# ehgus8/alpha-zero

Measured on AMD Instinct MI355X. Metric: selfplay_games_per_sec, higher is better.
Workload: dtype bf16

## Files before the change

alpha-zero_amd/azk/__init__.py:

```python
import ctypes as C
import math
import os
import subprocess

import numpy as np

_HERE = os.path.dirname(os.path.abspath(__file__))
_CSRC = os.path.join(os.path.dirname(_HERE), "csrc")
LIB_PATH = os.path.join(_HERE, "libazk.so")

ABI_VERSION = 4

SYMBOLS = [
    "azk_abi_version", "azk_last_error", "azk_create", "azk_destroy", "azk_geometry", "azk_reset_games",
    "azk_set_positions", "azk_begin_search", "azk_step_select", "azk_step_expand_backup", "azk_step",
    "azk_root_stats", "azk_root_children", "azk_export_tree", "azk_advance", "azk_get_positions",
    "azk_get_counters", "azk_reset_counters", "azk_check_device_error", "azk_gen_noise",
    "azk_rules_legal_moves", "azk_rules_legal_mask", "azk_rules_apply_move", "azk_rules_undo_move",
    "azk_rules_check_winner", "azk_rules_canonical", "azk_softmax_rows",
    "azk_step_tree", "azk_step_gather", "azk_recycle_finished", "azk_nn_patch_embed", "azk_nn_cls_attention", "azk_nn_patch_embed_scores", "azk_nn_cls_pool", "azk_debug_stamps", "azk_debug_stamps_raw", "azk_emit_finished", "azk_clear_cache", "azk_nn_heads_finalize", "azk_nn_layernorm_rows",
    "azk_vanilla_set_rng", "azk_vanilla_get_rng", "azk_vanilla_search", "azk_nn_embed_pool",
    "azk_nn_gemm_rows", "azk_nn_layernorm_sum", "azk_nn_heads_finalize_sum", "azk_nn_ln_heads",
    "azk_leaf_source_of", "azk_nn_embed_pool_leaves", "azk_nn_embed_pool_compact", "azk_nn_embed_pool_compact_leaves",
    "azk_nn_embed_fold", "azk_nn_embed_fold_leaves", "azk_nnx_embed_fold", "azk_nnx_embed_fold_leaves",
# ... 54 lines not shown
    if not torch.cuda.is_available():
        raise AzkError("no GPU visible: the azk engine runs only on an MI355X (no CPU fallback)")
    return torch


def _stream():
    import torch
    return C.c_void_p(torch.cuda.current_stream().cuda_stream)


def _p(t):
    return C.c_void_p(t.data_ptr()) if t is not None else None


def _np(a):
    return a.ctypes.data_as(C.c_void_p) if a is not None else None


def _ok(rc, name):
    if rc != 0:
        raise AzkError(f"{name} failed ({rc})")


class Engine:

    def __init__(self, game, n_games, max_sims, size=None, device=0, leaf_dtype="float32", arena_nodes=0, cache_entries=0,
                 cache_shared=False, leaves_per_step=1, tree_reuse=0):
        torch = _torch()
        self.torch = torch
        self.L = lib()
        self.game = game
        cfg = Config()
        cfg.game = GAME_ID[game]
        cfg.rows = cfg.cols = int(size or 0)
        cfg.n_games, cfg.max_sims, cfg.device, cfg.arena_nodes = int(n_games), int(max_sims), int(device), int(arena_nodes)
        cfg.cache_entries = int(cache_entries)
        cfg.cache_shared = 1 if (cache_shared and cache_entries) else 0
        self.cache_shared = bool(cfg.cache_shared)
        self.K = max(1, int(leaves_per_step))
        cfg.leaves_per_step = self.K
        self.tree_reuse = int(tree_reuse)
        cfg.tree_reuse = self.tree_reuse
        cfg.leaf_dtype = LEAF_BF16 if leaf_dtype in ("bfloat16", "bf16", torch.bfloat16) else LEAF_F32
        self.device = torch.device("cuda", device)
        torch.cuda.set_device(self.device)
        h = C.c_void_p()
        rc = self.L.azk_create(C.byref(cfg), C.byref(h))
        if rc != 0:
            raise AzkError(f"azk_create failed ({rc}): {self.L.azk_last_error(None).decode()}")
        self.h = h
        vals = [C.c_int32() for _ in range(5)]
        self._chk(self.L.azk_geometry(self.h, *[C.byref(v) for v in vals]))
        self.planes, self.rows, self.cols, self.action_dim, self.state_dim = [v.value for v in vals]
        self.G, self.max_sims = int(n_games), int(max_sims)
        tdt = torch.bfloat16 if cfg.leaf_dtype == LEAF_BF16 else torch.float32
        dev = self.device
        self.slots = self.G * self.K
        self.leaf_boards = torch.zeros((self.slots, self.planes, self.rows, self.cols), dtype=tdt, device=dev)
        self.n_leaf = torch.zeros(1, dtype=torch.int32, device=dev)
        self.pi = torch.zeros((self.G, self.action_dim), dtype=torch.float64, device=dev)
        self.q = torch.zeros(self.G, dtype=torch.float64, device=dev)
        self.root_visit = torch.zeros(self.G, dtype=torch.int32, device=dev)
        self.chosen = torch.zeros(self.G, dtype=torch.int32, device=dev)
        self.winner = torch.zeros(self.G, dtype=torch.int32, device=dev)
        self.done = torch.zeros(self.G, dtype=torch.int32, device=dev)
        self._noise = None
        self.cache_entries = int(cache_entries)
# ... 795 lines not shown
```

alpha-zero_amd/csrc/azk_device.h:

```cpp
#pragma once
#include <hip/hip_runtime.h>
#include <stdint.h>

#define AZK_WAVE 64
#define AZK_KIND_TTT 0
#define AZK_KIND_C4 1
#define AZK_KIND_GOMOKU 2

struct GameDesc {
    int kind, rows, cols, rc, planes, win_len, action_dim, state_dim;
    unsigned inv_cols;
};

__device__ __forceinline__ int azk_action_idx(const GameDesc &g, int cell) {
    return g.kind == AZK_KIND_C4 ? cell % g.cols : cell;
}

__device__ __forceinline__ int azk_lane() { return threadIdx.x & 63; }

__device__ __forceinline__ int uniform_i32(int v) { return __builtin_amdgcn_readfirstlane(v); }

__device__ __forceinline__ void azk_wave_sync() {
    __builtin_amdgcn_fence(__ATOMIC_RELEASE, "wavefront");
    __builtin_amdgcn_wave_barrier();
// ... 148 lines not shown

__device__ __forceinline__ unsigned long long py_tuple2_hash(int r, int c) {
    const unsigned long long P1 = 11400714785074694791ULL, P2 = 14029467366897019727ULL, P5 = 2870177450012600261ULL;
    unsigned long long acc = P5;
    acc += (unsigned long long)r * P2; acc = (acc << 31) | (acc >> 33); acc *= P1;
    acc += (unsigned long long)c * P2; acc = (acc << 31) | (acc >> 33); acc *= P1;
    acc += 2ULL ^ (P5 ^ 3527539ULL);
    if (acc == ~0ULL) return 1546275796ULL;
    return acc;
}

struct MoveScratch {
    uint32_t *bits;
    uint16_t *pref;
    int16_t *ord;
    uint16_t *tabA, *tabB;
    uint32_t *claim;
    int table_size;
};

struct AzkNoHook { __device__ __forceinline__ void operator()() const {} };

__device__ __forceinline__ int azk_valid_moves_small(const uint8_t *b, const GameDesc &g, int16_t *moves) {
    const int lane = azk_lane();
    int n = 0;
    if (g.kind == AZK_KIND_TTT) {
        for (int base = 0; base < g.rc; base += AZK_WAVE) {
            int i = base + lane;
            bool emp = i < g.rc && b[i] == 0;
            unsigned long long m = __ballot(emp);
            if (emp) moves[n + __popcll(m & ((1ull << lane) - 1ull))] = (int16_t)i;
            n += __popcll(m);
        }
        __syncthreads();
        return n;
    }
    int cell = -1;
    if (lane < g.cols && b[lane] == 0) {
        for (int row = g.rows - 1; row >= 0; row--)
            if (b[row * g.cols + lane] == 0) { cell = row * g.cols + lane; break; }
    }
    unsigned long long m = __ballot(cell >= 0);
    if (cell >= 0) moves[__popcll(m & ((1ull << lane) - 1ull))] = (int16_t)cell;
    __syncthreads();
    return __popcll(m);
}

template <int KMAX = 7, typename Mid = AzkNoHook>
__device__ int azk_valid_moves_gomoku(const uint8_t *b, const GameDesc &g, int16_t *moves, const MoveScratch &ms, bool skip_set = false,
                                      long long *dbgv = nullptr, Mid &&mid = Mid()) {
    const int lane = azk_lane();
    int n = 0;
    const int R = g.rows, C = g.cols, rc = g.rc;
    const int nwords = (rc * 8 + 31) >> 5;
    long long s0 = dbgv ? clock64() : 0, s1 = 0, s2 = 0, s3 = 0;
    const unsigned inv = g.inv_cols;
    uint8_t code[KMAX];
#pragma unroll
    for (int k = 0; k < KMAX; k++) {
        const int e = lane + AZK_WAVE * k;
        code[k] = b[e < rc ? e : 0];
    }
    for (int w = lane; w < nwords; w += AZK_WAVE) ms.bits[w] = 0u;
    unsigned long long S[KMAX + 1], CL[KMAX], CR[KMAX];
    bool empty[KMAX];
#pragma unroll
    for (int k = 0; k < KMAX; k++) {
        S[k] = 0ull; CL[k] = 0ull; CR[k] = 0ull; empty[k] = false;
        if (AZK_WAVE * k >= rc) continue;
        const int e = lane + AZK_WAVE * k;
        const bool in = e < rc;
        const int r = (int)(((unsigned)(in ? e : 0) * inv) >> 16), c = (in ? e : 0) - r * C;
        S[k] = __ballot(in && (code[k] & 3));
        CL[k] = __ballot(c >= 1);
        CR[k] = __ballot(c <= C - 2);
        empty[k] = in && code[k] == 0;
    }
// ... 315 lines not shown
```

alpha-zero_amd/csrc/azk_engine.hip:

```cpp
#include <hip/hip_runtime.h>
#include <hip/hip_bf16.h>
#include <stdint.h>
#include <stdio.h>
#include <stdlib.h>
#include <string.h>
#include <string>
#include <vector>

#include "azk.h"
#include "azk_device.h"

namespace {

enum { CNT_SIMS = 0, CNT_SCANNED, CNT_TRACE, CNT_CREATED, CNT_LEAVES, CNT_TERMINAL, CNT_MOVES, CNT_CACHE_HITS, CNT_REUSED, CNT_CARRIED, CNT_N };

struct __attribute__((aligned(16))) NodeH { int N; float P; uint32_t meta; int fc; };
typedef float f32x4_a4 __attribute__((ext_vector_type(4), aligned(4)));

struct Dev {
    GameDesc g;
    int G, cap, path_cap, rc_pad, leaf_dtype, table_size, lds_bytes;
    int lds_off[12];
    int K;
    uint8_t *cells;
// ... 19 lines not shown
    int cache_shared;
    unsigned long long cache_mask;
    unsigned *cache_claim;
    unsigned *cache_stamp;
    unsigned long long *leaf_key;
    float *hit_logits, *hit_value;
    int16_t *traj_action;
    double *traj_pi;
    long long *emit_base;
    int *sims_done;
    int *budget;
    long long *counters;
    int *err;
    int ablate;
    long long *dbg;
};

struct ReuseDev {
    int mode;
    int words;
    int *chosen_node;
    unsigned long long *bits;
    unsigned *pre;
};

struct LdsView {
    uint8_t *board;
    int *path;
    int16_t *moves;
    float *e;
    int *cnt;
    double *cdf;
    MoveScratch ms;
};

__host__ __device__ inline int up16(int x) { return (x + 15) & ~15; }

__host__ __device__ inline int lds_layout(const GameDesc &g, int path_cap, int table_size, int *off) {
    int o = 0;
    off[0] = o; o += up16(g.rc);
    off[1] = o; o += up16(path_cap * 4);
    off[2] = o; o += up16(g.rc * 2);
    int ea = g.action_dim > g.rc ? g.action_dim : g.rc;
    off[3] = o; o += up16(ea * 4);
    off[4] = o; o += up16(ea * 4);
    off[5] = o; o += up16(ea * 8);
    int nwords = (g.rc * 8 + 31) >> 5;
    off[6] = o; o += up16((nwords > (table_size >> 5) + 2 ? nwords : (table_size >> 5) + 2) * 4);
    off[7] = o; o += up16(nwords * 2);
    off[8] = o; o += up16(g.rc * 2);
    off[9] = o; o += up16(table_size * 2);
    off[10] = o; o += up16(table_size * 2);
    off[11] = o; o += up16(table_size * 4);
    return o;
}

extern __shared__ __attribute__((aligned(16))) unsigned char azk_smem[];

__device__ __forceinline__ LdsView carve_at(const int *off, int table_size) {
    LdsView L;
    L.board = azk_smem + off[0];
    L.path = (int *)(azk_smem + off[1]);
    L.moves = (int16_t *)(azk_smem + off[2]);
    L.e = (float *)(azk_smem + off[3]);
    L.cnt = (int *)(azk_smem + off[4]);
    L.cdf = (double *)(azk_smem + off[5]);
    L.ms.bits = (uint32_t *)(azk_smem + off[6]);
    L.ms.pref = (uint16_t *)(azk_smem + off[7]);
    L.ms.ord = (int16_t *)(azk_smem + off[8]);
    L.ms.tabA = (uint16_t *)(azk_smem + off[9]);
    L.ms.tabB = (uint16_t *)(azk_smem + off[10]);
    L.ms.claim = (uint32_t *)(azk_smem + off[11]);
    L.ms.table_size = table_size;
    return L;
}

__device__ __forceinline__ LdsView carve(const GameDesc &g, int path_cap, int table_size) {
    int off[12];
    lds_layout(g, path_cap, table_size, off);
    LdsView L;
    L.board = azk_smem + off[0];
    L.path = (int *)(azk_smem + off[1]);
    L.moves = (int16_t *)(azk_smem + off[2]);
    L.e = (float *)(azk_smem + off[3]);
    L.cnt = (int *)(azk_smem + off[4]);
    L.cdf = (double *)(azk_smem + off[5]);
    L.ms.bits = (uint32_t *)(azk_smem + off[6]);
    L.ms.pref = (uint16_t *)(azk_smem + off[7]);
    L.ms.ord = (int16_t *)(azk_smem + off[8]);
    L.ms.tabA = (uint16_t *)(azk_smem + off[9]);
    L.ms.tabB = (uint16_t *)(azk_smem + off[10]);
    L.ms.claim = (uint32_t *)(azk_smem + off[11]);
    L.ms.table_size = table_size;
    return L;
}

__device__ __forceinline__ uint32_t meta_pack(int cell, int nch) { return ((uint32_t)(cell & 0xffff) << 16) | (uint32_t)nch; }
__device__ __forceinline__ int meta_cell(uint32_t m) { return (int)(m >> 16); }
__device__ __forceinline__ int meta_nch(uint32_t m) { return (int)(m & 0xffffu); }

__device__ __forceinline__ void count_add(const Dev &d, int which, int g, long long v) {
    atomicAdd((unsigned long long *)&d.counters[(size_t)which * d.G + g], (unsigned long long)v);
}

__device__ __forceinline__ void backup_path(const Dev &d, size_t base, const int *path, int depth, double value, bool undo_virtual_loss = false) {
    for (int i = azk_lane(); i <= depth; i += AZK_WAVE) {
        int nd = path[i];
        double sv = ((depth - i) & 1) ? -value : value;
        if (undo_virtual_loss) { d.W[base + nd] = (d.W[base + nd] + sv) + 1.0; continue; }
        d.H[base + nd].N += 1;
        d.W[base + nd] += sv;
    }
}

template <bool EXPAND, bool SELECT, bool DBG, bool MULTI = false, int KSL = 7>
__global__ __launch_bounds__(AZK_WAVE) void k_tree(Dev dd, const float *__restrict__ logits, const float *__restrict__ values) {
    const Dev &d = dd;
    const int ablate = DBG ? dd.ablate : 0;
    const int g = blockIdx.x;
    const int lane0 = azk_lane();
    const GameDesc &gd = d.g;
    const int A = gd.action_dim, rc = gd.rc;
    const size_t base = (size_t)g * (size_t)d.cap;
    LdsView L = carve_at(d.lds_off, d.table_size);
    const bool wrec = DBG && (ablate & 8192) != 0;
    const bool stamp = (ablate & 16) != 0 || wrec;
    long long t0 = stamp ? clock64() : 0, t1 = 0, t2 = 0, t3 = 0, t4 = 0;
    int rec_type = -1, rec_depth = 0, rec_nv = 0, rec_env = 0;
    int done_sims = MULTI ? d.sims_done[g] : 0;
    const int sim_target = MULTI ? d.budget[0] : 0, max_iter = MULTI ? d.budget[1] : 1;
    const int young = MULTI ? d.budget[2] : 0;
    const long long t_launch = MULTI && young > 0 ? (long long)wall_clock64() : 0;
    auto still_young = [&]() { return young <= 0 || (long long)wall_clock64() - t_launch < (long long)young; };
    for (int it = 0; it < max_iter; it++) {
    int lane = lane0;
    if (MULTI) asm volatile("" : "+v"(lane));
    if (MULTI && it > 0) __syncthreads();
    const bool vl = MULTI && d.K > 1;
    const int vi = g * d.K + (vl ? it : 0);

    const bool shared = d.cache_entries && d.cache_shared;
    int e_node, e_slot, e_depth, e_nv, e_top, e_centry, s_done, s_player, s_mc, s_rootf64, r_fc, r_N;
    uint32_t r_meta;
    unsigned cstamp;
    constexpr bool ONE_LOAD = EXPAND && SELECT && !MULTI;
    int uw = 0;
    if (ONE_LOAD) {
        const int *up = d.leaf_node + vi;
        up = lane == 1 ? d.leaf_slot + vi : up;
        up = lane == 2 ? d.leaf_depth + vi : up;
        up = lane == 3 ? d.leaf_nmoves + vi : up;
        up = lane == 4 ? d.arena_top + g : up;
        up = (lane == 5 && d.cache_entries) ? d.leaf_cache + vi : up;
        up = (lane == 6 && shared) ? (const int *)d.cache_stamp : up;
        up = lane == 7 ? d.done + g : up;
        up = lane == 8 ? d.to_move + g : up;
        up = lane == 9 ? d.move_count + g : up;
        up = lane == 10 ? d.root_f64 + g : up;
        up = lane == 11 ? &d.H[base].fc : up;
        up = lane == 12 ? &d.H[base].N : up;
        up = lane == 13 ? (const int *)&d.H[base].meta : up;
        uw = *up;
    } else {
        e_node = EXPAND ? d.leaf_node[vi] : -1; e_slot = EXPAND ? d.leaf_slot[vi] : 0; e_depth = EXPAND ? d.leaf_depth[vi] : 0;
        e_nv = EXPAND ? d.leaf_nmoves[vi] : 0; e_top = EXPAND ? d.arena_top[g] : 0;
        e_centry = (EXPAND && d.cache_entries) ? d.leaf_cache[vi] : -1;
        cstamp = shared ? d.cache_stamp[0] : 0u;
        s_done = SELECT ? d.done[g] : 1; s_player = SELECT ? d.to_move[g] : 0; s_mc = SELECT ? d.move_count[g] : 0;
        s_rootf64 = SELECT ? d.root_f64[g] : 0;
        r_fc = SELECT ? d.H[base].fc : -1; r_N = SELECT ? d.H[base].N : 0;
        r_meta = SELECT ? d.H[base].meta : 0u;
    }
    unsigned long long e_key = 0ull;
    if (EXPAND && shared) e_key = d.leaf_key[(size_t)vi * d.key_words + min(lane, d.key_words - 1)];
    const int e_path = EXPAND ? d.path[(size_t)vi * d.path_cap + min(lane, d.path_cap - 1)] : 0;
    int e_mv[KSL] = {};
    if (EXPAND) {
#pragma unroll
        for (int k4 = 0; k4 < KSL; k4++) e_mv[k4] = d.leaf_moves[(size_t)vi * rc + min(lane + AZK_WAVE * k4, rc - 1)];
    }
    constexpr int NCW = (KSL * AZK_WAVE / 4 + AZK_WAVE - 1) / AZK_WAVE;
    const int ncw = d.rc_pad >> 2;
    uint32_t s_cw[NCW] = {};
    if (SELECT) {
        const uint32_t *cw = (const uint32_t *)(d.cells + (size_t)g * d.rc_pad);
#pragma unroll
        for (int q = 0; q < NCW; q++) s_cw[q] = cw[min(lane + AZK_WAVE * q, ncw - 1)];
    }
    if (ONE_LOAD) {
        e_node = __builtin_amdgcn_readlane(uw, 0); e_slot = __builtin_amdgcn_readlane(uw, 1); e_depth = __builtin_amdgcn_readlane(uw, 2);
        e_nv = __builtin_amdgcn_readlane(uw, 3); e_top = __builtin_amdgcn_readlane(uw, 4);
        e_centry = d.cache_entries ? __builtin_amdgcn_readlane(uw, 5) : -1;
        cstamp = shared ? (unsigned)__builtin_amdgcn_readlane(uw, 6) : 0u;
        s_done = __builtin_amdgcn_readlane(uw, 7); s_player = __builtin_amdgcn_readlane(uw, 8); s_mc = __builtin_amdgcn_readlane(uw, 9);
        s_rootf64 = __builtin_amdgcn_readlane(uw, 10); r_fc = __builtin_amdgcn_readlane(uw, 11); r_N = __builtin_amdgcn_readlane(uw, 12);
        r_meta = (uint32_t)__builtin_amdgcn_readlane(uw, 13);
    }

    if (EXPAND) {
        const int node = uniform_i32(e_node);
        if (MULTI && node >= 0 && !(d.cache_entries && uniform_i32(e_centry) >= 0) && ((!vl && it > 0) || logits == nullptr)) {
            if (lane == 0) atomicExch(d.err, AZK_ERR_STATE);
            break;
        }
        if (node >= 0) {
            const bool xst = (ablate & 1024) != 0;
            long long x0 = 0, x1 = 0, x2 = 0, x3 = 0, x4 = 0;
            if (xst) { asm volatile("s_waitcnt vmcnt(0)" ::: "memory"); x0 = clock64(); }
            const int slot = uniform_i32(e_slot);
            const int depth = uniform_i32(e_depth);
            const int nv = uniform_i32(e_nv);
            if (wrec) rec_env = nv;
            const int centry = d.cache_entries ? uniform_i32(e_centry) : -1;
            const bool hit = d.cache_entries && centry >= 0;
            const size_t crow = shared ? (size_t)(hit ? centry : -(centry + 1)) : ((size_t)g * d.cache_entries + (hit ? centry : -(centry + 1)));
            const float *lg = hit ? (shared ? d.hit_logits + (size_t)vi * A : d.cache_logits + crow * A) : logits + (size_t)slot * A;
            unsigned claim_now = 0u;
            if (shared && !hit) claim_now = __hip_atomic_load(d.cache_claim + crow, __ATOMIC_RELAXED, __HIP_MEMORY_SCOPE_AGENT);
            const bool shortpath = depth < AZK_WAVE;
            const int bnode = (shortpath && lane <= depth) ? e_path : 0;
            const int bN = d.H[base + bnode].N;
            const double bW = d.W[base + bnode];
            constexpr int NV4 = (KSL * AZK_WAVE + 255) / 256;
            int la[NV4];
            bool lact[NV4];
            f32x4_a4 lgv[NV4];
#pragma unroll
            for (int q = 0; q < NV4; q++) {
                lact[q] = 256 * q + 4 * lane < A;
                la[q] = min(256 * q + 4 * lane, A - 4);
                lgv[q] = *(const f32x4_a4 *)(lg + la[q]);
            }
            const float vraw = hit ? (shared ? d.hit_value[vi] : d.cache_value[crow]) : values[slot];
            const uint32_t node_meta = d.H[base + node].meta;
// ... 74 lines not shown
            if (xst && lane == 0) {
                x4 = clock64();
                long long *qq = d.dbg + (size_t)g * 8;
                qq[0] += x0 - t0; qq[1] += x1 - x0; qq[2] += x2 - x1; qq[3] += x3 - x2; qq[4] += x4 - x3; qq[6] += 1;
            }
            if (lane == 0) {
                d.leaf_node[vi] = -1;
                count_add(d, CNT_TRACE, g, depth + 1);
            }
        }
        azk_wave_sync();
    }

    if (SELECT) {
        const bool active = uniform_i32(s_done) == 0;
        if (!active || (MULTI && done_sims >= sim_target)) {
            if (lane == 0 && (!MULTI || it == 0 || vl)) d.leaf_flag[vi] = 0;
            if (vl) continue;
            break;
        }
        done_sims++;
        if (stamp) t1 = clock64();
#pragma unroll
        for (int q = 0; q < NCW; q++) { const int i = lane + AZK_WAVE * q; if (i < ncw) ((uint32_t *)L.board)[i] = s_cw[q]; }
        const int root_player = uniform_i32(s_player);
        const int root_mc = uniform_i32(s_mc);
        if (lane == 0) L.path[0] = 0;
        azk_wave_sync();
        int node = 0, depth = 0, scanned = 0;
        int fc = uniform_i32(r_fc);
        int Np = uniform_i32(r_N);
        uint32_t nmeta = (uint32_t)uniform_i32((int)r_meta);
        int node_cell = -1;
        const bool root_f64 = uniform_i32(s_rootf64) != 0;
        long long seg_a = 0, seg_b = 0, seg_c = 0, seg_d = 0, seg_t = 0;
        for (;;) {
            const int nch = meta_nch(nmeta);
            if (nch <= 0 || (ablate & 2)) break;
            if (ablate & 64) seg_t = clock64();
            const bool f64 = node == 0 && root_f64;
            double bu64 = 0.0;
            float bu32 = 0.f;
            int best = 0x7fffffff, bN = 0, bfc = -1;
            uint32_t bmeta = 0;
            if (nch <= AZK_WAVE && !(ablate & 2048)) {
                const bool valid = lane < nch;
                const size_t ci = base + fc + (valid ? lane : 0);
                const NodeH hc = d.H[ci];
                const double Wc = d.W[ci];
                const int Nc = hc.N, fcc = hc.fc;
                const uint32_t mc = hc.meta;
                const float P32 = hc.P;
                unsigned long long winners;
                if (f64) {
                    const double P64 = d.rootP[(size_t)g * rc + (valid ? lane : 0)];
                    const double s = sqrt((double)Np);
                    const double u0 = P64 * s / (double)(Nc + 1);
                    const double q = Wc / (double)Nc;
                    const double u = valid ? (Nc != 0 ? q + u0 : u0) : -__builtin_huge_val();
                    const double um = wave_max_f64(u);
                    winners = __ballot(valid & (u == um));
                } else {
                    const float s = (float)sqrt((double)Np);
                    const float u0 = (P32 * s) / (float)(Nc + 1);
                    const float q = (float)(Wc / (double)Nc);
                    const float u = valid ? (Nc != 0 ? q + u0 : u0) : -__builtin_huge_valf();
                    const float um = wave_max_f32(u);
                    winners = __ballot(valid & (u == um));
                }
// ... 90 lines not shown
            }
            const int wl = best & 63;
            scanned += nch;
            const int child = fc + best;
            Np = __builtin_amdgcn_readlane(bN, wl);
            nmeta = (uint32_t)__builtin_amdgcn_readlane((int)bmeta, wl);
            fc = __builtin_amdgcn_readlane(bfc, wl);
            if (ablate & 64) { const long long tn = clock64(); seg_c += tn - seg_t; seg_t = tn; }
            const int cellc = meta_cell(nmeta);
            const int mover = (root_player + depth) & 1;
            depth++;
            node = child;
            node_cell = cellc;
            if (lane == 0) {
                L.path[depth] = node;
                if (gd.kind == AZK_KIND_C4) L.board[cellc] |= (uint8_t)(1 << mover);
                else if (L.board[cellc] == 0) L.board[cellc] = (uint8_t)(1 << mover);
            }
            if (depth + 1 >= d.path_cap) break;
        }
        if ((ablate & 64) && lane == 0) {
            long long *qq = d.dbg + (size_t)g * 8;
            qq[0] += seg_a; qq[1] += seg_b; qq[2] += seg_c; qq[3] += seg_d; qq[5] += depth; qq[6] += 1;
        }
        azk_wave_sync();
        if (stamp) t2 = clock64();
        if (vl && fc == -2) {
            done_sims--;
            if (lane == 0) d.leaf_flag[vi] = 0;
            continue;
        }
        const int node_player = (root_player + depth) & 1;
        const int node_mc = root_mc + depth;
        int term = -1;
        if (depth > 0) {
            const int w = azk_check_winner(L.board, gd, 1 - node_player, node_cell);
            if (w != -1) term = 1;
            else if (node_mc == gd.state_dim) term = 0;
        }
        if (lane == 0) {
            count_add(d, CNT_SIMS, g, 1);
            count_add(d, CNT_SCANNED, g, scanned);
        }
        if (wrec) rec_depth = depth;
        if (term >= 0) {
            if (wrec) { rec_type = 0; t3 = t4 = clock64(); }
            backup_path(d, base, L.path, depth, (double)term);
            if (lane == 0) {
                d.leaf_flag[vi] = 0;
                count_add(d, CNT_TERMINAL, g, 1);
                count_add(d, CNT_TRACE, g, depth + 1);
            }
            if (MULTI && (vl || still_young())) continue;
            break;
        }
        if (stamp) t3 = clock64();
        bool cached = false;
        int entry = 0;
        unsigned long long mykey = 0ull, kw = 0ull;
        unsigned c1v = 0u, c2v = 0u;
        constexpr int NV4P = (KSL * AZK_WAVE + 255) / 256;
        f32x4_a4 row[NV4P] = {};
        float vv = 0.f;
        bool maybe_hit = false;
        const int KW = d.key_words;
        if (d.cache_entries) {
            const int half = KW >> 1;
            unsigned long long h = 0x9E3779B97F4A7C15ull;
            for (int q = 0; q < half; q++) {
                const int c = q * AZK_WAVE + lane;
                const uint8_t code = c < rc ? L.board[c] : (uint8_t)0;
                unsigned long long own = __ballot((code >> node_player) & 1);
                const unsigned long long opp = __ballot((code >> (node_player ^ 1)) & 1);
                if (q == half - 1) own |= (unsigned long long)node_player << 63;
                if (lane == q) mykey = own;
                if (lane == half + q) mykey = opp;
                h = (h ^ own) * 0xFF51AFD7ED558CCDull; h ^= h >> 29;
                h = (h ^ opp) * 0xC4CEB9FE1A85EC53ull; h ^= h >> 32;
            }
            if (shared) {
                entry = (int)(h & d.cache_mask);
                c1v = __hip_atomic_load(d.cache_claim + entry, __ATOMIC_RELAXED, __HIP_MEMORY_SCOPE_AGENT);
                kw = d.cache_key[(size_t)entry * KW + min(lane, KW - 1)];
#pragma unroll
                for (int q = 0; q < NV4P; q++) row[q] = *(const f32x4_a4 *)(d.cache_logits + (size_t)entry * A + min(256 * q + 4 * lane, A - 4));
                vv = d.cache_value[entry];
            } else {
                entry = (int)(h & (unsigned long long)(d.cache_entries - 1));
                kw = d.cache_key[((size_t)g * d.cache_entries + entry) * KW + min(lane, KW - 1)];
            }
        }
        auto probe_mid = [&]() {
            if (!(d.cache_entries && shared)) return;
            asm volatile("s_waitcnt vmcnt(0)" ::: "memory");
            const unsigned c1 = (unsigned)uniform_i32((int)c1v);
            const bool same = lane < KW ? kw == mykey : true;
            maybe_hit = c1 != 0u && c1 < cstamp && __ballot(!same) == 0ull;
            if (maybe_hit) c2v = __hip_atomic_load(d.cache_claim + entry, __ATOMIC_RELAXED, __HIP_MEMORY_SCOPE_AGENT);
        };
        int nv;
        unsigned c2 = 0u;
        if (ablate & 4) { nv = 1; if (lane == 0) L.moves[0] = (int16_t)(gd.rc / 2); __syncthreads(); probe_mid(); c2 = (unsigned)uniform_i32((int)c2v); }
        else if (gd.kind == AZK_KIND_GOMOKU) {
            nv = azk_valid_moves_gomoku<KSL>(L.board, gd, L.moves, L.ms, (ablate & 8) != 0, (ablate & 32) ? d.dbg + (size_t)g * 8 : nullptr, probe_mid);
            c2 = (unsigned)uniform_i32((int)c2v);
        } else { probe_mid(); c2 = (unsigned)uniform_i32((int)c2v); nv = azk_valid_moves_small(L.board, gd, L.moves); }
        if (stamp) t4 = clock64();
        if (d.cache_entries) {
            if (shared) {
                if (maybe_hit && c2 == (unsigned)uniform_i32((int)c1v)) {
                    cached = true;
#pragma unroll
                    for (int q = 0; q < NV4P; q++) if (256 * q + 4 * lane < A) *(f32x4_a4 *)(d.hit_logits + (size_t)vi * A + min(256 * q + 4 * lane, A - 4)) = row[q];
                    if (lane == 0) d.hit_value[vi] = vv;
                }
                if (!cached && lane < KW) d.leaf_key[(size_t)vi * KW + lane] = mykey;
            } else {
                unsigned long long *kp = d.cache_key + ((size_t)g * d.cache_entries + entry) * KW;
                const bool same = lane < KW ? kw == mykey : true;
                cached = __ballot(!same) == 0ull;
                if (!cached && lane < KW) kp[lane] = mykey;
            }
            if (lane == 0) d.leaf_cache[vi] = cached ? entry : -(entry + 1);
        }
        for (int i = lane; i < nv; i += AZK_WAVE) d.leaf_moves[(size_t)vi * rc + i] = L.moves[i];
        {
            uint32_t *lw = (uint32_t *)(d.leaf_cells + (size_t)vi * d.rc_pad);
#pragma unroll
            for (int q = 0; q < NCW; q++) { const int i = lane + AZK_WAVE * q; if (i < ncw) lw[i] = ((const uint32_t *)L.board)[i]; }
        }
        for (int i = lane; i <= depth; i += AZK_WAVE) d.path[(size_t)vi * d.path_cap + i] = L.path[i];
        if (vl) {
            for (int i = lane; i <= depth; i += AZK_WAVE) { const int nd = L.path[i]; d.H[base + nd].N += 1; d.W[base + nd] -= 1.0; }
            if (lane == 0) d.H[base + node].fc = -2;
        }
        if (lane == 0) {
            d.leaf_node[vi] = node; d.leaf_depth[vi] = depth; d.leaf_nmoves[vi] = nv;
            d.leaf_flag[vi] = cached ? 0 : (uint8_t)(1 + min(7, node_mc / 6));
            if (cached) count_add(d, CNT_CACHE_HITS, g, 1);
            count_add(d, CNT_LEAVES, g, cached ? 0 : 1);
            if (wrec) { rec_type = cached ? 1 : 2; rec_nv = nv; }
            if (stamp && !wrec) {
                long long *q = d.dbg + (size_t)g * 8;
                const long long tend = clock64();
                q[0] += t1 - t0; q[1] += t2 - t1; q[2] += t3 - t2; q[3] += t4 - t3; q[4] += tend - t4; q[5] += depth; q[6] += 1;
                if (!(ablate & 64) && tend - t0 > q[7]) q[7] = tend - t0;
            }
        }
        if (MULTI && (vl || (cached && still_young()))) continue;
    }
    if (vl) continue;
    break;
    }
    if (MULTI && lane0 == 0) d.sims_done[g] = done_sims;
    if (wrec) {
        asm volatile("s_waitcnt vmcnt(0)" ::: "memory");
        if (lane0 == 0) {
            long long *q = d.dbg + (size_t)g * 8;
            const long long tend = clock64();
            if (rec_type < 0) { t1 = t2 = t3 = t4 = tend; }
            q[0] = t1 - t0; q[1] = t2 - t1; q[2] = t3 - t2; q[3] = t4 - t3; q[4] = tend - t4; q[5] = rec_depth;
            q[6] = (long long)(rec_type + 1) | ((long long)rec_nv << 8) | ((long long)rec_env << 20); q[7] = tend - t0;
        }
    }
}

#define AZK_LAUNCH_TREE(E_, S_, D_, M_, ARGS_) do { \
        if (d.g.rc <= 4 * AZK_WAVE && d.g.action_dim <= 4 * AZK_WAVE) k_tree<E_, S_, D_, M_, 4><<<d.G, AZK_WAVE, d.lds_bytes, st>>> ARGS_; \
        else k_tree<E_, S_, D_, M_, 7><<<d.G, AZK_WAVE, d.lds_bytes, st>>> ARGS_; } while (0)

__global__ __launch_bounds__(AZK_WAVE) void k_gather(Dev d, void *__restrict__ leaf_boards, int *__restrict__ n_leaf_out) {
    const int g = blockIdx.x, lane = azk_lane();
    const int NV = d.G * d.K;
    int before = 0, total = 0;
    const unsigned long long *fw = (const unsigned long long *)d.leaf_flag;
    const int nw = (NV + 7) >> 3;
    const bool last = g == NV - 1;
    const int limit_words = last ? nw : ((g + 8) >> 3);
    for (int w0 = 0; w0 < limit_words; w0 += AZK_WAVE) {
        int w = w0 + lane;
        unsigned long long x = w < nw ? fw[w] : 0ull;
        x = (((x & 0x7f7f7f7f7f7f7f7full) + 0x7f7f7f7f7f7f7f7full) | x) & 0x8080808080808080ull;
        total += __popcll(x);
        int lo = w * 8;
        if (lo + 8 <= g) before += __popcll(x);
        else if (lo < g) before += __popcll(x & ((1ull << ((g - lo) * 8)) - 1ull));
    }
    before = wave_sum_i32(before);
    if (last) {
        total = wave_sum_i32(total);
        if (lane == 0) {
            *n_leaf_out = total;
            if (d.cache_entries && d.cache_shared) d.cache_stamp[0] += 1u;
        }
    }
    if (!d.leaf_flag[g]) return;
    const int slot = before;
    if (lane == 0) d.leaf_slot[g] = slot;
    const int rc = d.g.rc, F = d.g.planes;
    const int player = (d.to_move[g / d.K] + d.leaf_depth[g]) & 1;
    const uint8_t *b = d.leaf_cells + (size_t)g * d.rc_pad;
    const size_t o = (size_t)slot * F * rc;
// ... 1564 lines not shown
```

Baseline: 1017.

## Split tree kernel into two waves overlapping expansion with next selection

The non-multi tree kernel now launches two wavefronts per game. The second wave expands the previous leaf (softmax of logits, child creation, cache write, move generation) while the first wave backs up values and starts the next selection, joining at a workgroup barrier only when selection reaches the just-expanded node. Cache probing is issued before the terminal check to hide its latency. Block-wide syncs in small-game move generation become wavefront syncs. This adds LDS for a second board and a handoff area, plus barrier coordination, and relies on the leaf-node reset for correctness.

```diff
diff --git a/alpha-zero_amd/azk/__init__.py b/alpha-zero_amd/azk/__init__.py
--- a/alpha-zero_amd/azk/__init__.py
+++ b/alpha-zero_amd/azk/__init__.py
@@ -110,7 +110,7 @@
         self.game = game
         cfg = Config()
         cfg.game = GAME_ID[game]
-        cfg.rows = cfg.cols = int(size or 0)
+        cfg.rows, cfg.cols = (int(size[0]), int(size[1])) if isinstance(size, (tuple, list)) else (int(size or 0), int(size or 0))
         cfg.n_games, cfg.max_sims, cfg.device, cfg.arena_nodes = int(n_games), int(max_sims), int(device), int(arena_nodes)
         cfg.cache_entries = int(cache_entries)
         cfg.cache_shared = 1 if (cache_shared and cache_entries) else 0
diff --git a/alpha-zero_amd/csrc/azk_device.h b/alpha-zero_amd/csrc/azk_device.h
--- a/alpha-zero_amd/csrc/azk_device.h
+++ b/alpha-zero_amd/csrc/azk_device.h
@@ -204,7 +204,7 @@
             if (emp) moves[n + __popcll(m & ((1ull << lane) - 1ull))] = (int16_t)i;
             n += __popcll(m);
         }
-        __syncthreads();
+        azk_wave_sync();
         return n;
     }
     int cell = -1;
@@ -214,7 +214,7 @@
     }
     unsigned long long m = __ballot(cell >= 0);
     if (cell >= 0) moves[__popcll(m & ((1ull << lane) - 1ull))] = (int16_t)cell;
-    __syncthreads();
+    azk_wave_sync();
     return __popcll(m);
 }
 
diff --git a/alpha-zero_amd/csrc/azk_engine.hip b/alpha-zero_amd/csrc/azk_engine.hip
--- a/alpha-zero_amd/csrc/azk_engine.hip
+++ b/alpha-zero_amd/csrc/azk_engine.hip
@@ -75,6 +75,8 @@
     int *cnt;
     double *cdf;
     MoveScratch ms;
+    uint8_t *board1;
+    int *ho;
 };
 
 __host__ __device__ inline int up16(int x) { return (x + 15) & ~15; }
@@ -95,12 +97,14 @@
     off[9] = o; o += up16(table_size * 2);
     off[10] = o; o += up16(table_size * 2);
     off[11] = o; o += up16(table_size * 4);
+    off[12] = o; o += up16(g.rc);
+    off[13] = o; o += 32;
     return o;
 }
 
 extern __shared__ __attribute__((aligned(16))) unsigned char azk_smem[];
 
-__device__ __forceinline__ LdsView carve_at(const int *off, int table_size) {
+__device__ __forceinline__ LdsView carve_at(const int *off, int table_size, int rc) {
     LdsView L;
     L.board = azk_smem + off[0];
     L.path = (int *)(azk_smem + off[1]);
@@ -115,11 +119,14 @@
     L.ms.tabB = (uint16_t *)(azk_smem + off[10]);
     L.ms.claim = (uint32_t *)(azk_smem + off[11]);
     L.ms.table_size = table_size;
+    const int o12 = off[11] + up16(table_size * 4);
+    L.board1 = azk_smem + o12;
+    L.ho = (int *)(azk_smem + o12 + up16(rc));
     return L;
 }
 
 __device__ __forceinline__ LdsView carve(const GameDesc &g, int path_cap, int table_size) {
-    int off[12];
+    int off[14];
     lds_layout(g, path_cap, table_size, off);
     LdsView L;
     L.board = azk_smem + off[0];
@@ -135,6 +142,8 @@
     L.ms.tabB = (uint16_t *)(azk_smem + off[10]);
     L.ms.claim = (uint32_t *)(azk_smem + off[11]);
     L.ms.table_size = table_size;
+    L.board1 = azk_smem + off[12];
+    L.ho = (int *)(azk_smem + off[13]);
     return L;
 }
 
@@ -156,8 +165,166 @@
     }
 }
 
+__device__ __forceinline__ int row_first(int wanted, int A) { return max(min(wanted, A - 4), 0); }
+__device__ __forceinline__ f32x4_a4 row_load4(const float *row, int first, int A) {
+    if (A >= 4) return *(const f32x4_a4 *)(row + first);
+    f32x4_a4 v;
+#pragma unroll
+    for (int c = 0; c < 4; c++) v[c] = row[min(first + c, A - 1)];
+    return v;
+}
+__device__ __forceinline__ void row_store4(float *row, int first, int A, f32x4_a4 v) {
+    if (A >= 4) { *(f32x4_a4 *)(row + first) = v; return; }
+#pragma unroll
+    for (int c = 0; c < 4; c++) if (first + c < A) row[first + c] = v[c];
+}
+
+enum { HO_OK = 0, HO_FC, HO_NV, HO_ROOTF64, HO_END_LO, HO_END_HI };
+
+template <bool DBG, int KSL>
+__device__ __forceinline__ void tree_expand_wave(const Dev &d, const LdsView &L, const float *__restrict__ logits, const float *__restrict__ values, int ablate) {
+    const int g = blockIdx.x, vi = g * d.K, lane = azk_lane();
+    const GameDesc &gd = d.g;
+    const int A = gd.action_dim, rc = gd.rc;
+    const size_t base = (size_t)g * (size_t)d.cap;
+    const bool shared = d.cache_entries && d.cache_shared;
+    const bool wrec = DBG && (ablate & 8192) != 0;
+    const int *up = d.leaf_node + vi;
+    up = lane == 1 ? d.leaf_slot + vi : up;
+    up = lane == 2 ? d.leaf_depth + vi : up;
+    up = lane == 3 ? d.leaf_nmoves + vi : up;
+    up = lane == 4 ? d.arena_top + g : up;
+    up = (lane == 5 && d.cache_entries) ? d.leaf_cache + vi : up;
+    up = (lane == 6 && shared) ? (const int *)d.cache_stamp : up;
+    const int uw = *up;
+    unsigned long long e_key = 0ull;
+    if (shared) e_key = d.leaf_key[(size_t)vi * d.key_words + min(lane, d.key_words - 1)];
+    constexpr int NCW = (KSL * AZK_WAVE / 4 + AZK_WAVE - 1) / AZK_WAVE;
+    const int ncw = d.rc_pad >> 2;
+    uint32_t cw[NCW];
+    {
+        const uint32_t *lw = (const uint32_t *)(d.leaf_cells + (size_t)vi * d.rc_pad);
+#pragma unroll
+        for (int q = 0; q < NCW; q++) cw[q] = lw[min(lane + AZK_WAVE * q, ncw - 1)];
+    }
+    const int node = __builtin_amdgcn_readlane(uw, 0);
+    int ok = 0, fc = -1, nv = 0, rootf64 = 0;
+    if (node >= 0) {
+        const bool xst = (ablate & 1024) != 0;
+        long long x0 = 0, x1 = 0, x2 = 0, x3 = 0, x4 = 0;
+        if (xst) { asm volatile("s_waitcnt vmcnt(0)" ::: "memory"); x0 = clock64(); }
+        const int slot = __builtin_amdgcn_readlane(uw, 1);
+        const int depth = __builtin_amdgcn_readlane(uw, 2);
+        nv = __builtin_amdgcn_readlane(uw, 3);
+        const int centry = d.cache_entries ? __builtin_amdgcn_readlane(uw, 5) : -1;
+        const unsigned cstamp = shared ? (unsigned)__builtin_amdgcn_readlane(uw, 6) : 0u;
+        const bool hit = d.cache_entries && centry >= 0;
+        const size_t crow = shared ? (size_t)(hit ? centry : -(centry + 1)) : ((size_t)g * d.cache_entries + (hit ? centry : -(centry + 1)));
+        const float *lg = hit ? (shared ? d.hit_logits + (size_t)vi * A : d.cache_logits + crow * A) : logits + (size_t)slot * A;
+        unsigned claim_now = 0u;
+        if (shared && !hit) claim_now = __hip_atomic_load(d.cache_claim + crow, __ATOMIC_RELAXED, __HIP_MEMORY_SCOPE_AGENT);
+        constexpr int NV4 = (KSL * AZK_WAVE + 255) / 256;
+        int la[NV4];
+        bool lact[NV4];
+        f32x4_a4 lgv[NV4];
+#pragma unroll
+        for (int q = 0; q < NV4; q++) {
+            lact[q] = 256 * q + 4 * lane < A;
+            la[q] = row_first(256 * q + 4 * lane, A);
+            lgv[q] = row_load4(lg, la[q], A);
+        }
+        const float vraw = hit ? (shared ? d.hit_value[vi] : d.cache_value[crow]) : values[slot];
+        const uint32_t node_meta = d.H[base + node].meta;
+#pragma unroll
+        for (int q = 0; q < NCW; q++) { const int i = lane + AZK_WAVE * q; if (i < ncw) ((uint32_t *)L.board1)[i] = cw[q]; }
+        if (nv >= 0) {
+            for (int i = lane; i < nv; i += AZK_WAVE) L.moves[i] = d.leaf_moves[(size_t)vi * rc + i];
+        }
+        azk_wave_sync();
+        if (nv < 0) {
+            if (ablate & 4) { nv = 1; if (lane == 0) L.moves[0] = (int16_t)(gd.rc / 2); azk_wave_sync(); }
+            else if (gd.kind == AZK_KIND_GOMOKU)
+                nv = azk_valid_moves_gomoku<KSL>(L.board1, gd, L.moves, L.ms, (ablate & 8) != 0, (ablate & 32) ? d.dbg + (size_t)g * 8 : nullptr);
+            else nv = azk_valid_moves_small(L.board1, gd, L.moves);
+        }
+        nv = uniform_i32(nv);
+        int e_mv[KSL];
+#pragma unroll
+        for (int k4 = 0; k4 < KSL; k4++) { const int i = lane + AZK_WAVE * k4; e_mv[k4] = L.moves[i < nv ? i : 0]; }
+        const bool mix = depth == 0 && d.noise != nullptr;
+        double nzv[KSL] = {};
+        if (mix) {
+#pragma unroll
+            for (int k4 = 0; k4 < KSL; k4++) nzv[k4] = d.noise[(size_t)g * A + azk_action_idx(gd, e_mv[k4])];
+        }
+        bool cache_write = d.cache_entries && !hit;
+        if (shared && !hit) {
+            const unsigned cur = (unsigned)uniform_i32((int)claim_now);
+            unsigned got = cur;
+            if (cur != cstamp && lane == 0) got = atomicCAS(d.cache_claim + crow, cur, cstamp);
+            cache_write = cur != cstamp && (unsigned)uniform_i32((int)got) == cur;
+            if (cache_write && lane < d.key_words) d.cache_key[crow * d.key_words + lane] = e_key;
+        }
+        if (xst) { asm volatile("s_waitcnt vmcnt(0)" ::: "memory"); x1 = clock64(); }
+#pragma unroll
+        for (int q = 0; q < NV4; q++) {
+            if (256 * q >= A) break;
+#pragma unroll
+            for (int c = 0; c < 4; c++) {
+                const float ev = (ablate & 1) ? 1.0f : azk_exp_det(lgv[q][c]);
+                if (lact[q] && la[q] + c < A) L.e[la[q] + c] = ev;
+            }
+        }
+        azk_wave_sync();
+        if (cache_write) {
+#pragma unroll
+            for (int q = 0; q < NV4; q++) if (lact[q]) row_store4(d.cache_logits + crow * A, la[q], A, lgv[q]);
+            if (lane == 0) d.cache_value[crow] = vraw;
+        }
+        if (xst) x2 = clock64();
+        const float s = azk_pairwise_sum(L.e, A);
+        if (xst) x3 = clock64();
+        fc = __builtin_amdgcn_readlane(uw, 4);
+        const bool fits = fc + nv <= d.cap;
+        if (fits) {
+#pragma unroll
+            for (int k4 = 0; k4 < KSL; k4++) {
+                const int i = lane + AZK_WAVE * k4;
+                if (i >= nv) break;
+                const int cell = e_mv[k4];
+                const int a = azk_action_idx(gd, cell);
+                const float p = L.e[a] / s;
+                const size_t idx = base + fc + i;
+                d.H[idx] = NodeH{0, p, meta_pack(cell, 0), -1}; d.W[idx] = 0.0;
+                if (mix) d.rootP[(size_t)g * rc + i] = (double)(0.75f * p) + 0.25 * nzv[k4];
+            }
+            if (lane == 0) {
+                d.H[base + node].fc = fc;
+                d.H[base + node].meta = (node_meta & 0xffff0000u) | (uint32_t)nv;
+                d.arena_top[g] = fc + nv;
+                if (depth == 0) d.root_f64[g] = mix ? 1 : 0;
+                count_add(d, CNT_CREATED, g, nv);
+            }
+            ok = 1; rootf64 = mix ? 1 : 0;
+        } else if (lane == 0) {
+            atomicExch(d.err, AZK_ERR_ARENA_FULL);
+        }
+        if (xst && lane == 0) {
+            x4 = clock64();
+            long long *qq = d.dbg + (size_t)g * 8;
+            qq[1] += x1 - x0; qq[2] += x2 - x1; qq[3] += x3 - x2; qq[4] += x4 - x3; qq[6] += 1;
+        }
+    }
+    if (wrec) asm volatile("s_waitcnt vmcnt(0)" ::: "memory");
+    if (lane == 0) {
+        L.ho[HO_OK] = ok; L.ho[HO_FC] = fc; L.ho[HO_NV] = nv; L.ho[HO_ROOTF64] = rootf64;
+        if (wrec) { const unsigned long long te = (unsigned long long)clock64(); L.ho[HO_END_LO] = (int)(unsigned)te; L.ho[HO_END_HI] = (int)(unsigned)(te >> 32); }
+    }
+}
+
+
 template <bool EXPAND, bool SELECT, bool DBG, bool MULTI = false, int KSL = 7>
-__global__ __launch_bounds__(AZK_WAVE) void k_tree(Dev dd, const float *__restrict__ logits, const float *__restrict__ values) {
+__global__ __launch_bounds__(MULTI ? AZK_WAVE : 2 * AZK_WAVE) void k_tree(Dev dd, const float *__restrict__ logits, const float *__restrict__ values) {
     const Dev &d = dd;
     const int ablate = DBG ? dd.ablate : 0;
     const int g = blockIdx.x;
@@ -165,11 +332,32 @@
     const GameDesc &gd = d.g;
     const int A = gd.action_dim, rc = gd.rc;
     const size_t base = (size_t)g * (size_t)d.cap;
-    LdsView L = carve_at(d.lds_off, d.table_size);
+    LdsView L = carve_at(d.lds_off, d.table_size, d.g.rc);
     const bool wrec = DBG && (ablate & 8192) != 0;
     const bool stamp = (ablate & 16) != 0 || wrec;
     long long t0 = stamp ? clock64() : 0, t1 = 0, t2 = 0, t3 = 0, t4 = 0;
-    int rec_type = -1, rec_depth = 0, rec_nv = 0, rec_env = 0;
+    constexpr bool TWO = !MULTI;
+    if constexpr (TWO) {
+        if (uniform_i32((int)(threadIdx.x >> 6)) != 0) {
+            if constexpr (EXPAND) tree_expand_wave<DBG, KSL>(d, L, logits, values, ablate);
+            asm volatile("s_waitcnt vmcnt(0)" ::: "memory");
+            __builtin_amdgcn_fence(__ATOMIC_RELEASE, "workgroup");
+            __builtin_amdgcn_s_barrier();
+            return;
+        }
+    }
+    bool joined = false;
+    int prev_leaf_done = -1;
+    int bar_phase = 0, prev_leaf_rec = -1;
+    long long bar_wait = 0, w1_end = 0;
+    auto join = [&](int phase) {
+        const long long ta = wrec ? clock64() : 0;
+        __builtin_amdgcn_s_barrier();
+        __builtin_amdgcn_fence(__ATOMIC_ACQUIRE, "workgroup");
+        if (wrec) { bar_wait += clock64() - ta; bar_phase = phase; }
+        joined = true;
+    };
+    int rec_type = -1, rec_depth = 0, rec_env = 0;
     int done_sims = MULTI ? d.sims_done[g] : 0;
     const int sim_target = MULTI ? d.budget[0] : 0, max_iter = MULTI ? d.budget[1] : 1;
     const int young = MULTI ? d.budget[2] : 0;
@@ -215,10 +403,10 @@
         r_meta = SELECT ? d.H[base].meta : 0u;
     }
     unsigned long long e_key = 0ull;
-    if (EXPAND && shared) e_key = d.leaf_key[(size_t)vi * d.key_words + min(lane, d.key_words - 1)];
+    if (EXPAND && MULTI && shared) e_key = d.leaf_key[(size_t)vi * d.key_words + min(lane, d.key_words - 1)];
     const int e_path = EXPAND ? d.path[(size_t)vi * d.path_cap + min(lane, d.path_cap - 1)] : 0;
     int e_mv[KSL] = {};
-    if (EXPAND) {
+    if (EXPAND && MULTI) {
 #pragma unroll
         for (int k4 = 0; k4 < KSL; k4++) e_mv[k4] = d.leaf_moves[(size_t)vi * rc + min(lane + AZK_WAVE * k4, rc - 1)];
     }
@@ -240,9 +428,44 @@
         r_meta = (uint32_t)__builtin_amdgcn_readlane(uw, 13);
     }
 
-    if (EXPAND) {
+    const int prev_leaf = (EXPAND && TWO) ? uniform_i32(e_node) : -1;
+    prev_leaf_done = prev_leaf;
+    if (wrec) prev_leaf_rec = prev_leaf;
+    int prev_crow = -1;
+    if constexpr (EXPAND && TWO) {
+        const int node = prev_leaf;
+        if (node >= 0) {
+            const int slot = uniform_i32(e_slot);
+            const int depth = uniform_i32(e_depth);
+            const int centry = d.cache_entries ? uniform_i32(e_centry) : -1;
+            const bool hit = d.cache_entries && centry >= 0;
+            const size_t crow = shared ? (size_t)(hit ? centry : -(centry + 1)) : ((size_t)g * d.cache_entries + (hit ? centry : -(centry + 1)));
+            if (shared && !hit) prev_crow = -(centry + 1);
+            const bool shortpath = depth < AZK_WAVE;
+            const int bnode = (shortpath && lane <= depth) ? e_path : 0;
+            const int bN = d.H[base + bnode].N;
+            const double bW = d.W[base + bnode];
+            const float vraw = hit ? (shared ? d.hit_value[vi] : d.cache_value[crow]) : values[slot];
+            const double v = -(double)vraw;
+            if (shortpath) {
+                const int nN = bN + 1;
+                const double nW = bW + (((depth - lane) & 1) ? -v : v);
+                if (lane <= depth) {
+                    d.H[base + e_path].N = nN;
+                    d.W[base + e_path] = nW;
+                }
+            } else {
+                backup_path(d, base, d.path + (size_t)vi * d.path_cap, depth, v, false);
+            }
+            r_N += 1;
+            if (lane == 0) count_add(d, CNT_TRACE, g, depth + 1);
+        }
+        azk_wave_sync();
+    }
+    if constexpr (EXPAND && MULTI) {
         const int node = uniform_i32(e_node);
-        if (MULTI && node >= 0 && !(d.cache_entries && uniform_i32(e_centry) >= 0) && ((!vl && it > 0) || logits == nullptr)) {
+        if (MULTI && node >= 0 && (uniform_i32(e_nv) < 0 ||
+                                   (!(d.cache_entries && uniform_i32(e_centry) >= 0) && ((!vl && it > 0) || logits == nullptr)))) {
             if (lane == 0) atomicExch(d.err, AZK_ERR_STATE);
             break;
         }
@@ -383,9 +606,16 @@
         int Np = uniform_i32(r_N);
         uint32_t nmeta = (uint32_t)uniform_i32((int)r_meta);
         int node_cell = -1;
-        const bool root_f64 = uniform_i32(s_rootf64) != 0;
+        bool root_f64 = uniform_i32(s_rootf64) != 0;
         long long seg_a = 0, seg_b = 0, seg_c = 0, seg_d = 0, seg_t = 0;
         for (;;) {
+            if (TWO && EXPAND && node == prev_leaf && !joined) {
+                join(1);
+                if (uniform_i32(L.ho[HO_OK])) {
+                    fc = uniform_i32(L.ho[HO_FC]); nmeta = (nmeta & 0xffff0000u) | (uint32_t)uniform_i32(L.ho[HO_NV]);
+                    if (node == 0) root_f64 = uniform_i32(L.ho[HO_ROOTF64]) != 0;
+                }
+            }
             const int nch = meta_nch(nmeta);
             if (nch <= 0 || (ablate & 2)) break;
             if (ablate & 64) seg_t = clock64();
@@ -542,29 +772,6 @@
         }
         const int node_player = (root_player + depth) & 1;
         const int node_mc = root_mc + depth;
-        int term = -1;
-        if (depth > 0) {
-            const int w = azk_check_winner(L.board, gd, 1 - node_player, node_cell);
-            if (w != -1) term = 1;
-            else if (node_mc == gd.state_dim) term = 0;
-        }
-        if (lane == 0) {
-            count_add(d, CNT_SIMS, g, 1);
-            count_add(d, CNT_SCANNED, g, scanned);
-        }
-        if (wrec) rec_depth = depth;
-        if (term >= 0) {
-            if (wrec) { rec_type = 0; t3 = t4 = clock64(); }
-            backup_path(d, base, L.path, depth, (double)term);
-            if (lane == 0) {
-                d.leaf_flag[vi] = 0;
-                count_add(d, CNT_TERMINAL, g, 1);
-                count_add(d, CNT_TRACE, g, depth + 1);
-            }
-            if (MULTI && (vl || still_young())) continue;
-            break;
-        }
-        if (stamp) t3 = clock64();
         bool cached = false;
         int entry = 0;
         unsigned long long mykey = 0ull, kw = 0ull;
@@ -574,7 +781,8 @@
         float vv = 0.f;
         bool maybe_hit = false;
         const int KW = d.key_words;
-        if (d.cache_entries) {
+        auto probe_issue = [&]() {
+            if (!d.cache_entries) return;
             const int half = KW >> 1;
             unsigned long long h = 0x9E3779B97F4A7C15ull;
             for (int q = 0; q < half; q++) {
@@ -593,35 +801,69 @@
                 c1v = __hip_atomic_load(d.cache_claim + entry, __ATOMIC_RELAXED, __HIP_MEMORY_SCOPE_AGENT);
                 kw = d.cache_key[(size_t)entry * KW + min(lane, KW - 1)];
 #pragma unroll
-                for (int q = 0; q < NV4P; q++) row[q] = *(const f32x4_a4 *)(d.cache_logits + (size_t)entry * A + min(256 * q + 4 * lane, A - 4));
+                for (int q = 0; q < NV4P; q++) {
+                    if constexpr (TWO) row[q] = row_load4(d.cache_logits + (size_t)entry * A, row_first(256 * q + 4 * lane, A), A);
+                    else row[q] = *(const f32x4_a4 *)(d.cache_logits + (size_t)entry * A + min(256 * q + 4 * lane, A - 4));
+                }
                 vv = d.cache_value[entry];
             } else {
                 entry = (int)(h & (unsigned long long)(d.cache_entries - 1));
                 kw = d.cache_key[((size_t)g * d.cache_entries + entry) * KW + min(lane, KW - 1)];
             }
-        }
+        };
+        if (TWO) probe_issue();
+        int term = -1;
+        if (depth > 0) {
+            const int w = azk_check_winner(L.board, gd, 1 - node_player, node_cell);
+            if (w != -1) term = 1;
+            else if (node_mc == gd.state_dim) term = 0;
+        }
+        if (lane == 0) {
+            count_add(d, CNT_SIMS, g, 1);
+            count_add(d, CNT_SCANNED, g, scanned);
+        }
+        if (wrec) rec_depth = depth;
+        if (term >= 0) {
+            if (wrec) { rec_type = 0; t3 = t4 = clock64(); }
+            backup_path(d, base, L.path, depth, (double)term);
+            if (lane == 0) {
+                d.leaf_flag[vi] = 0;
+                count_add(d, CNT_TERMINAL, g, 1);
+                count_add(d, CNT_TRACE, g, depth + 1);
+            }
+            if (MULTI && (vl || still_young())) continue;
+            break;
+        }
+        if (stamp) t3 = clock64();
+        if (MULTI) probe_issue();
         auto probe_mid = [&]() {
             if (!(d.cache_entries && shared)) return;
             asm volatile("s_waitcnt vmcnt(0)" ::: "memory");
             const unsigned c1 = (unsigned)uniform_i32((int)c1v);
             const bool same = lane < KW ? kw == mykey : true;
             maybe_hit = c1 != 0u && c1 < cstamp && __ballot(!same) == 0ull;
+            if (TWO && entry == prev_crow) maybe_hit = false;
             if (maybe_hit) c2v = __hip_atomic_load(d.cache_claim + entry, __ATOMIC_RELAXED, __HIP_MEMORY_SCOPE_AGENT);
         };
-        int nv;
+        int nv = -1;
         unsigned c2 = 0u;
-        if (ablate & 4) { nv = 1; if (lane == 0) L.moves[0] = (int16_t)(gd.rc / 2); __syncthreads(); probe_mid(); c2 = (unsigned)uniform_i32((int)c2v); }
+        if constexpr (TWO) { probe_mid(); c2 = (unsigned)uniform_i32((int)c2v); }
         else if (gd.kind == AZK_KIND_GOMOKU) {
-            nv = azk_valid_moves_gomoku<KSL>(L.board, gd, L.moves, L.ms, (ablate & 8) != 0, (ablate & 32) ? d.dbg + (size_t)g * 8 : nullptr, probe_mid);
+            nv = azk_valid_moves_gomoku<KSL>(L.board, gd, L.moves, L.ms, false, nullptr, probe_mid);
             c2 = (unsigned)uniform_i32((int)c2v);
         } else { probe_mid(); c2 = (unsigned)uniform_i32((int)c2v); nv = azk_valid_moves_small(L.board, gd, L.moves); }
         if (stamp) t4 = clock64();
+        if (TWO && !joined) join(2);
+        prev_leaf_done = -1;
         if (d.cache_entries) {
             if (shared) {
                 if (maybe_hit && c2 == (unsigned)uniform_i32((int)c1v)) {
                     cached = true;
 #pragma unroll
-                    for (int q = 0; q < NV4P; q++) if (256 * q + 4 * lane < A) *(f32x4_a4 *)(d.hit_logits + (size_t)vi * A + min(256 * q + 4 * lane, A - 4)) = row[q];
+                    for (int q = 0; q < NV4P; q++) if (256 * q + 4 * lane < A) {
+                        if constexpr (TWO) row_store4(d.hit_logits + (size_t)vi * A, row_first(256 * q + 4 * lane, A), A, row[q]);
+                        else *(f32x4_a4 *)(d.hit_logits + (size_t)vi * A + min(256 * q + 4 * lane, A - 4)) = row[q];
+                    }
                     if (lane == 0) d.hit_value[vi] = vv;
                 }
                 if (!cached && lane < KW) d.leaf_key[(size_t)vi * KW + lane] = mykey;
@@ -633,7 +875,7 @@
             }
             if (lane == 0) d.leaf_cache[vi] = cached ? entry : -(entry + 1);
         }
-        for (int i = lane; i < nv; i += AZK_WAVE) d.leaf_moves[(size_t)vi * rc + i] = L.moves[i];
+        if (MULTI) for (int i = lane; i < nv; i += AZK_WAVE) d.leaf_moves[(size_t)vi * rc + i] = L.moves[i];
         {
             uint32_t *lw = (uint32_t *)(d.leaf_cells + (size_t)vi * d.rc_pad);
 #pragma unroll
@@ -649,7 +891,7 @@
             d.leaf_flag[vi] = cached ? 0 : (uint8_t)(1 + min(7, node_mc / 6));
             if (cached) count_add(d, CNT_CACHE_HITS, g, 1);
             count_add(d, CNT_LEAVES, g, cached ? 0 : 1);
-            if (wrec) { rec_type = cached ? 1 : 2; rec_nv = nv; }
+            if (wrec) rec_type = cached ? 1 : 2;
             if (stamp && !wrec) {
                 long long *q = d.dbg + (size_t)g * 8;
                 const long long tend = clock64();
@@ -663,21 +905,30 @@
     break;
     }
     if (MULTI && lane0 == 0) d.sims_done[g] = done_sims;
+    if (TWO && !joined) join(3);
+    if (TWO && EXPAND && prev_leaf_done >= 0 && lane0 == 0) d.leaf_node[g * d.K] = -1;
     if (wrec) {
         asm volatile("s_waitcnt vmcnt(0)" ::: "memory");
         if (lane0 == 0) {
             long long *q = d.dbg + (size_t)g * 8;
             const long long tend = clock64();
             if (rec_type < 0) { t1 = t2 = t3 = t4 = tend; }
-            q[0] = t1 - t0; q[1] = t2 - t1; q[2] = t3 - t2; q[3] = t4 - t3; q[4] = tend - t4; q[5] = rec_depth;
-            q[6] = (long long)(rec_type + 1) | ((long long)rec_nv << 8) | ((long long)rec_env << 20); q[7] = tend - t0;
+            if (EXPAND && prev_leaf_rec >= 0) {
+                rec_env = L.ho[HO_OK] ? L.ho[HO_NV] : 0;
+                w1_end = (long long)(((unsigned long long)(unsigned)L.ho[HO_END_HI] << 32) | (unsigned)L.ho[HO_END_LO]);
+            }
+            const long long w1 = (prev_leaf_rec >= 0 && w1_end > t0) ? w1_end - t0 : 0;
+            q[0] = t1 - t0; q[1] = t2 - t1; q[2] = t3 - t2; q[3] = t4 - t3; q[4] = tend - t4;
+            q[5] = (long long)rec_depth | (bar_wait << 16) | ((long long)bar_phase << 56);
+            q[6] = (long long)(rec_type + 1) | ((long long)rec_env << 20) | (w1 << 32); q[7] = tend - t0;
         }
     }
 }
 
 #define AZK_LAUNCH_TREE(E_, S_, D_, M_, ARGS_) do { \
-        if (d.g.rc <= 4 * AZK_WAVE && d.g.action_dim <= 4 * AZK_WAVE) k_tree<E_, S_, D_, M_, 4><<<d.G, AZK_WAVE, d.lds_bytes, st>>> ARGS_; \
-        else k_tree<E_, S_, D_, M_, 7><<<d.G, AZK_WAVE, d.lds_bytes, st>>> ARGS_; } while (0)
+        const int nthr_ = (M_) ? AZK_WAVE : 2 * AZK_WAVE;               \
+        if (d.g.rc <= 4 * AZK_WAVE && d.g.action_dim <= 4 * AZK_WAVE) k_tree<E_, S_, D_, M_, 4><<<d.G, nthr_, d.lds_bytes, st>>> ARGS_; \
+        else k_tree<E_, S_, D_, M_, 7><<<d.G, nthr_, d.lds_bytes, st>>> ARGS_; } while (0)
 
 __global__ __launch_bounds__(AZK_WAVE) void k_gather(Dev d, void *__restrict__ leaf_boards, int *__restrict__ n_leaf_out) {
     const int g = blockIdx.x, lane = azk_lane();
```

Result: faster. 1090 (median of 6 runs) (+7.1%).
